# lisqzqng/Video-based-gait-analysis-for-dementia

Measured on AMD Instinct MI355X. Metric: frames/sec (224x224, seq=16), higher is better.
Workload: dtype f32

## Files before the change

video-based-gait-analysis-for-dementia_amd/csrc/conv_wino4.hip:

```cpp
#include "kernels.h"
#include "device.h"
#include "conv_wino4_tile.h"

#include <cstdio>
#include <cstdlib>

namespace grk {

namespace {

#ifdef GRNET_ABLATION
__device__ unsigned long long g_w4phase[8];
#endif

constexpr int kCK = 8;
constexpr size_t kLdsB = Wino4Geom<56, kCK, 256>::lds_bytes;

template <typename T>
__device__ __forceinline__ void landed(T& x) { asm volatile("" : "+v"(x)); }

template <int NB, int WD, int ABL, bool WSPLIT>
__device__ __forceinline__ void conv_wino4_body(const ConvArgs& a) {
    constexpr bool PAIR = NB == 2 && !WSPLIT;
    constexpr int NLD = PAIR ? 9 : 18;
// ... 175 lines not shown
                    if (has_add) y += rcur[i];
                    if (a.relu) { y[0] = fmaxf(y[0], 0.f); y[1] = fmaxf(y[1], 0.f); y[2] = fmaxf(y[2], 0.f); y[3] = fmaxf(y[3], 0.f); }
                    *reinterpret_cast<f32x4*>(a.out + obase + i * WD) = y;
                }
            }
        }
    }
    ticks.mark(3);
    ticks.count(4);
    ticks.flush(GRK_ABL_COUNTERS(g_w4phase), tid == 0);
}

template <int NB, int WD = 56, int ABL = 0, bool WSPLIT = false>
__global__ __launch_bounds__(256) void conv_wino4_f32(const ConvArgs a) { conv_wino4_body<NB, WD, ABL, WSPLIT>(a); }

constexpr int kCKW = 16;
constexpr size_t kLdsW = Wino4Geom<56, kCKW, 512>::lds_bytes;

template <int WD, int NPW>
__device__ __forceinline__ void conv_wino4w_body(const ConvArgs& a) {
    typedef Wino4Geom<WD, kCKW, 512> G;
    constexpr int TPR = G::TPR, TRG = G::TRG, kRawW = G::RAWW, UPC = G::UPC, kVW = G::V, kMrow = G::MROW;
    constexpr int COUTW = 2 * NPW * 16;
    static_assert(NPW == 4 || NPW == 2, "geometry");
    typedef float bfrag __attribute__((ext_vector_type(NPW)));
    extern __shared__ __align__(16) float smem[];
    float* raw = smem;
    float* V = raw + G::VOFF;
    const int tid = threadIdx.x, lane = tid & 63, wave = __builtin_amdgcn_readfirstlane(tid >> 6), l15 = lane & 15, lq = lane >> 4;
    const int pg = wave & 3, hf = wave >> 2;

    const int id = blockIdx.x;
    int img, r, by;
    G::decode(a, id, img, r, by);
    const int co0 = by * COUTW + hf * (NPW * 16);
    const int wpos = NPW == 4 ? co0 : (co0 & ~63) + ((co0 >> 5) & 1) * 2;
    set_wave_prio(a.prio);
    const int HW = a.H * a.W;
    const float* inb = a.in + ((size_t)img * a.in_ctot + a.in_coff) * HW;
    const int g0 = (4 * TRG * r - 1) * WD;

    const __amdgpu_buffer_rsrc_t u_rsrc = buffer_rsrc(a.w, 36 * a.CinPad * a.CoutPad * 4), r_rsrc = buffer_rsrc(inb, a.Cin * HW * 4);
    const int ub = ((pg * 9 * a.CinPad + lq) * a.CoutPad + wpos + l15 * 4) * 4;
    const int u_point = a.CinPad * a.CoutPad * 4, u_kstep = 4 * a.CoutPad * 4, u_chunk = kCKW * a.CoutPad * 4;
    auto load_u = [&](int chunk, int q, int e) -> bfrag {
        const int soff = chunk * u_chunk + (3 * (q >> 1) + (e >> 1)) * u_point + (2 * (q & 1) + (e & 1)) * u_kstep;
        if constexpr (NPW == 4) return __builtin_bit_cast(bfrag, __builtin_amdgcn_raw_buffer_load_b128(u_rsrc, ub, soff, 0));
        else return __builtin_bit_cast(bfrag, __builtin_amdgcn_raw_buffer_load_b64(u_rsrc, ub, soff, 0));
    };
    int roff[G::NRU];
#pragma unroll
    for (int i = 0; i < G::NRU; ++i) {
        const int u = i * G::NT + tid, ch = u / UPC, k = u - ch * UPC, gi = g0 + 4 * k;
        const bool unit = u < kCKW * UPC, inside = gi >= 0 && gi < HW;
        roff[i] = unit && inside ? (ch * HW + gi) * 4 : -1;
        if (unit && !inside) {
            *reinterpret_cast<f32x4*>(raw + u * 4) = f32x4{0.f, 0.f, 0.f, 0.f};
// ... 10 lines not shown
    const int vpos = (hf * 18) * (kCKW * 16) + chn * 16 + slot;
    auto transform = [&](const float* rp, float* vp) {
        Wino4Patch<G> t;
        t.read(rp);
        t.halo(real);
        t.rows(hf);
        t.cols(vp);
    };

    f32x4 acc[9][NPW];
#pragma unroll
    for (int p = 0; p < 9; ++p)
#pragma unroll
        for (int n = 0; n < NPW; ++n) acc[p][n] = f32x4{0.f, 0.f, 0.f, 0.f};

    const int nchunks = a.CinPad / kCKW;
    bfrag bq[6];
    float av[2][6];
    auto load_a = [&](int buf, int q, int set) {
#pragma unroll
        for (int e = 0; e < 6; ++e) {
            const int p = pg * 9 + 3 * (q >> 1) + (e >> 1), ks = 2 * (q & 1) + (e & 1);
            av[set][e] = V[buf * kVW + p * (kCKW * 16) + (ks * 4 + lq) * 16 + l15];
        }
    };
    auto multiply = [&](int buf, int ch, bool more) {
        load_a(buf, 0, 0);
#pragma unroll
        for (int q = 0; q < 6; ++q) {
#pragma unroll
            for (int e = 0; e < 6; ++e) landed(av[q & 1][e]);
// ... 1 lines not shown
            if (q < 5) load_a(buf, q + 1, (q + 1) & 1);
            __builtin_amdgcn_sched_barrier(0);
#pragma unroll
            for (int e = 0; e < 6; ++e) {
                const int pi = 3 * (q >> 1) + (e >> 1);
#pragma unroll
                for (int n = 0; n < NPW; ++n) acc[pi][n] = __builtin_amdgcn_mfma_f32_16x16x4f32(av[q & 1][e], bq[e][n], acc[pi][n], 0, 0, 0);
                __builtin_amdgcn_sched_barrier(0);
                if (q < 5) bq[e] = load_u(ch, q + 1, e);
                else if (more) bq[e] = load_u(ch + 1, 0, e);
                __builtin_amdgcn_sched_barrier(0);
            }
        }
    };

    const bool has_add = a.n_add == 1;
    const int eh = tid >> 8;
    typename G::Epi ep;
    G::epi(tid & 255, r, a.H, ep);
    f32x4 radd[4] = {f32x4{0.f, 0.f, 0.f, 0.f}, f32x4{0.f, 0.f, 0.f, 0.f}, f32x4{0.f, 0.f, 0.f, 0.f}, f32x4{0.f, 0.f, 0.f, 0.f}};
    auto fetch_res = [&](int nt) {
        const int co = by * COUTW + eh * (NPW * 16) + nt * 16 + ep.ec;
        if (has_add && ep.on && co < a.Cout) G::fetch_res(radd, a, ep, img, co, HW);
    };

    issue_raw(0);
    if (nchunks > 1) issue_raw(1);
#pragma unroll
    for (int e = 0; e < 6; ++e) bq[e] = load_u(0, 0, e);
    asm volatile("s_waitcnt vmcnt(6)" ::: "memory");
    __syncthreads();
// ... 30 lines not shown
        }
        __syncthreads();
        const f32x4 rcur[4] = {radd[0], radd[1], radd[2], radd[3]};
        if (nt + 1 < NPW) fetch_res(nt + 1);
        if (ep.on) {
            const int co = by * COUTW + eh * (NPW * 16) + nt * 16 + ep.ec;
            if (co < a.Cout) {
                float s4[4][6];
#pragma unroll
                for (int j = 0; j < 6; ++j) {
                    float m[6];
#pragma unroll
                    for (int i = 0; i < 6; ++i) m[i] = Mr[((i * 6 + j) * 16 + ep.ec) * kMrow + ep.et];
                    at_f43(m, s4[0][j], s4[1][j], s4[2][j], s4[3][j]);
                }
                const float b = a.bias[co];
                const size_t obase = ((size_t)img * a.out_ctot + a.out_coff + co) * HW + ep.eorow * WD + 4 * ep.etx;
#pragma unroll
                for (int i = 0; i < 4; ++i) {
                    float y0, y1, y2, y3;
                    at_f43<true>(s4[i], y0, y1, y2, y3, b);
                    f32x4 y = f32x4{y0, y1, y2, y3};
                    if (has_add) y += rcur[i];
                    if (a.relu) { y[0] = fmaxf(y[0], 0.f); y[1] = fmaxf(y[1], 0.f); y[2] = fmaxf(y[2], 0.f); y[3] = fmaxf(y[3], 0.f); }
                    *reinterpret_cast<f32x4*>(a.out + obase + i * WD) = y;
                }
            }
        }
    }
}

template <int WD, int NPW>
__global__ __launch_bounds__(512) void conv_wino4w_f32(const ConvArgs a) { conv_wino4w_body<WD, NPW>(a); }

}

int conv_wino4_wide(int cout, int w) {
    static const int wide_env = GRNET_AB(WINO_WIDE, 1);
    if (w == 56) return cout % 128 == 0 ? ((wide_env & 1) ? 4 : 0) : cout == 64 ? ((wide_env & 8) ? 2 : 0) : 0;
    if (w == 28) return cout % 128 == 0 ? ((wide_env & 4) ? 4 : 0) : cout == 64 ? ((wide_env & 2) ? 2 : 0) : 0;
    return 0;
}
int conv_wino4_blocks(int cout, int w) { return (cout % 64 == 0 && !(w == 28 && cout == 64 && !conv_wino4_wide(cout, w))) ? 4 : 2; }

bool conv_wino4_eligible(int cin, int cout, int ks, int stride, int h, int w, int n_add) {
    return ks == 3 && stride == 1 && ((h == 56 && w == 56) || (h == 28 && w == 28)) && n_add <= 1 && cin % kCK == 0 && cout % 32 == 0 && cin >= 32;
}

static size_t wino4_lds() {
    static const size_t pad = (size_t)GRNET_AB(WINO_LDS_PAD, 0);
    return kLdsB + pad;
}

hipError_t conv_wino4_form(const ConvArgs& a, Wino4Form* f) {
    *f = Wino4Form{};
    f->nb = conv_wino4_blocks(a.Cout, a.W);
    if (!conv_wino4_eligible(a.Cin, a.Cout, a.ks, a.stride, a.H, a.W, a.n_add) || a.CinPad % kCK != 0 || a.CoutPad % (f->nb * 16) != 0) return hipErrorInvalidValue;
    if (a.n_add == 1 && a.add_shift[0] != 0) return hipErrorInvalidValue;
    const int npw = conv_wino4_wide(a.Cout, a.W);
    const bool wide = npw && a.CinPad % kCKW == 0 && a.CoutPad % (npw * 32) == 0 && !(a.dbg & 32);
    const int trg = wino4_tile_rows(a.W);
    f->waves = wide ? 8 : 4;
    f->npw = wide ? npw : 0;
    f->gx = a.N * (((a.H >> 2) + trg - 1) / trg);
    f->gy = a.CoutPad / (wide ? npw * 32 : f->nb * 16);
    f->xcd = f->gx % 8 == 0 && f->gx >= 16 ? 1 : 0;
    const int total = f->gx * f->gy;
    f->full = total;
    if (wide || f->nb == 2) return hipSuccess;
    static const int split_env = GRNET_AB(WINO_SPLIT, 1);
    int kCUs = 0;
    if (hipError_t e = device_cu_count(&kCUs); e != hipSuccess) return e;
    const int full = total / kCUs * kCUs, rest = total - full;
    if (split_env && full > 0 && rest > 0 && 2 * rest <= kCUs && (!f->xcd || full % 8 == 0)) {
        f->split = 1;
        f->full = full;
        f->rest = rest;
    }
    return hipSuccess;
}

static void apply_form(ConvArgs& a, const Wino4Form& f, int* n_launches) {
    a.gx = f.gx;
    a.gy = f.gy;
// ... 18 lines not shown
        }
    }
#endif
    if (f.nb == 2) return launch_k(conv_wino4_f32<2, WD>, dim3(total), dim3(256), kLdsB, s, a);
    if (f.split) {
        hipError_t e = launch_k(conv_wino4_f32<4, WD>, dim3(f.full), dim3(256), kLdsB, s, a);
        if (e != hipSuccess) return e;
        a.blk0 = f.full;
        a.wsplit = 1;
        if (n_launches) *n_launches = 2;
        return launch_k(conv_wino4_f32<2, WD, 0, true>, dim3(2 * f.rest), dim3(256), kLdsB, s, a);
    }
    return launch_k(conv_wino4_f32<4, WD>, dim3(total), dim3(256), kLdsB, s, a);
}

hipError_t launch_conv_wino4(ConvArgs a, hipStream_t s, int* n_launches) {
    static PerDeviceOnce attr;
    int dev = 0;
    if (hipError_t e = current_device(&dev); e != hipSuccess) return e;
    if (hipError_t e = once_per_device(attr, dev, [](int*) {
            hipError_t e = hipSuccess;
            const size_t l4 = wino4_lds();
            auto set = [&](auto kern, size_t lds) { if (e == hipSuccess) e = hipFuncSetAttribute(reinterpret_cast<const void*>(kern), hipFuncAttributeMaxDynamicSharedMemorySize, (int)lds); };
            set(conv_wino4_f32<4, 56>, l4); set(conv_wino4_f32<2, 56>, l4); set(conv_wino4_f32<4, 28>, l4); set(conv_wino4_f32<2, 28>, l4);
            set(conv_wino4_f32<2, 56, 0, true>, l4); set(conv_wino4_f32<2, 28, 0, true>, l4);
            set(conv_wino4w_f32<56, 4>, kLdsW); set(conv_wino4w_f32<56, 2>, kLdsW); set(conv_wino4w_f32<28, 4>, kLdsW); set(conv_wino4w_f32<28, 2>, kLdsW);
            return e;
        }); e != hipSuccess) return e;
    Wino4Form f;
    if (hipError_t e = conv_wino4_form(a, &f); e != hipSuccess) return e;
    if (f.waves == 8) {
        apply_form(a, f, n_launches);
        const dim3 grid(a.gx * a.gy);
        if (a.W == 56) return f.npw == 4 ? launch_k(conv_wino4w_f32<56, 4>, grid, dim3(512), kLdsW, s, a) : launch_k(conv_wino4w_f32<56, 2>, grid, dim3(512), kLdsW, s, a);
        return f.npw == 4 ? launch_k(conv_wino4w_f32<28, 4>, grid, dim3(512), kLdsW, s, a) : launch_k(conv_wino4w_f32<28, 2>, grid, dim3(512), kLdsW, s, a);
    }
#ifdef GRNET_ABLATION
    if (GRNET_AB_SET(W4_PHASES)) {
        a.dbg |= 8;
        const hipError_t e = a.W == 56 ? launch_wino4_w<56>(a, s, f, n_launches) : launch_wino4_w<28>(a, s, f, n_launches);
        unsigned long long h[8] = {};
        abl::take_counters(HIP_SYMBOL(g_w4phase), h, s);
        const double n = h[4] ? (double)h[4] : 1.0;
        fprintf(stderr, "[wino4 phases] %d->%d @%d N%d add %d nb %d wgs %llu: per WG ticks  prologue %.0f  first transform %.0f  chunk loop %.0f (%d chunks)  epilogue %.0f\n",
                a.Cin, a.Cout, a.W, a.N, a.n_add, f.nb, h[4], h[0] / n, h[1] / n, h[2] / n, a.CinPad / kCK, h[3] / n);
        return e;
    }
// ... 34 lines not shown
```

video-based-gait-analysis-for-dementia_amd/csrc/grnet_hooks.cpp:

```cpp
#include "grnet_impl.h"

namespace {

struct HookBuffers {
    std::vector<void*> ptrs;
    HookBuffers() = default;
    HookBuffers(const HookBuffers&) = delete;
    HookBuffers& operator=(const HookBuffers&) = delete;
    ~HookBuffers() { for (void* p : ptrs) (void)hipFree(p); }
    template <class T = void>
    T* alloc(size_t bytes) {
        void* p = nullptr;
        if (hipMalloc(&p, bytes) != hipSuccess) return nullptr;
        ptrs.push_back(p);
        return static_cast<T*>(p);
    }
};

template <class F, class E>
float timed_launches(hipStream_t s, int reps, F&& launch, E* err) {
    hipEvent_t e0 = nullptr, e1 = nullptr;
    if (hipEventCreate(&e0) != hipSuccess || hipEventCreate(&e1) != hipSuccess) {
        if (e0) (void)hipEventDestroy(e0);
        return -1.f;
// ... 197 lines not shown
    if (hipMemcpy(wd, wp.data(), wp.size() * 4, hipMemcpyHostToDevice) != hipSuccess ||
        hipMemcpy(bd, bp.data(), bp.size() * 4, hipMemcpyHostToDevice) != hipSuccess)
        return h->fail(GRNET_EHIP, "hipMemcpy of the test weights failed");
    const int pad = ks / 2;
    ConvArgs a{};
    a.in = in_dev; a.in_ctot = cin; a.in_coff = 0; a.N = n; a.Cin = cin; a.H = hgt; a.W = wid;
    a.Cout = cout; a.Ho = (hgt + 2 * pad - ks) / stride + 1; a.Wo = (wid + 2 * pad - ks) / stride + 1;
    a.out = out_dev; a.out_ctot = cout; a.out_coff = 0;
    a.w = wd; a.bias = bd; a.CinPad = cin_pad; a.CoutPad = cout_pad; a.ks = ks; a.stride = stride; a.relu = relu;
    if (add_dev) { a.n_add = 1; a.add[0] = add_dev; a.add_ctot[0] = cout; a.add_coff[0] = 0; a.add_shift[0] = 0; }
    a.zeros = h->zeros;
    if (const char* d = GRNET_AB_STR(CONV_DBG)) a.dbg = atoi(d);
    hipStream_t s = static_cast<hipStream_t>(stream);
    float* ud = nullptr;
    if (tile_hint == 2003) { tile_hint = 2001; a.dbg |= 32; }
    if (tile_hint == 2001) {
        if (!conv_wino4_eligible(cin, cout, ks, stride, hgt, wid, add_dev ? 1 : 0) || cin_pad % 8 != 0 || cout_pad % (cout % 64 == 0 ? 64 : 32) != 0)
            return h->fail(GRNET_EINVAL, "shape not eligible for the F(4x4,3x3) kernel");
        std::vector<double> wf((size_t)cout * cin * 9);
        for (size_t i = 0; i < wf.size(); ++i) wf[i] = w_host[i];
        std::vector<float> uw((size_t)36 * cin_pad * cout_pad);
        pack_wino4_weights(wf.data(), cout, cin, cin_pad, cout_pad, uw.data(), wid);
        if (!(ud = mem.alloc<float>(uw.size() * 4)) || hipMemcpy(ud, uw.data(), uw.size() * 4, hipMemcpyHostToDevice) != hipSuccess)
            return h->fail(GRNET_ENOMEM, "Winograd test weights");
        a.w = ud;
    }
    if (tile_hint == 3002 && !conv_pw_eligible(cin, cout, ks, stride, hgt, wid, add_dev ? 1 : 0))
        return h->fail(GRNET_EINVAL, "shape not eligible for the 1x1 kernel");
    if (tile_hint == 3001) {
        if (!conv_stem_eligible(cin, cout, ks, stride, hgt, wid, add_dev ? 1 : 0))
            return h->fail(GRNET_EINVAL, "shape not eligible for the stem kernel");
        std::vector<double> wf((size_t)cout * cin * 9);
        for (size_t i = 0; i < wf.size(); ++i) wf[i] = w_host[i];
        std::vector<float> sw(7 * 4 * 64);
        pack_stem_weights(wf.data(), sw.data());
        if (!(ud = mem.alloc<float>(sw.size() * 4)) || hipMemcpy(ud, sw.data(), sw.size() * 4, hipMemcpyHostToDevice) != hipSuccess)
            return h->fail(GRNET_ENOMEM, "stem test weights");
        a.w = ud;
    }
    int w4s_on = 0, w4s_ks = 0;
    if (tile_hint >= 2020 && tile_hint <= 2024) {
        w4s_on = 1; w4s_ks = tile_hint - 2020;
        if (!conv_wino4s_eligible(cin, cout, ks, stride, hgt, wid, add_dev ? 1 : 0))
            return h->fail(GRNET_EINVAL, "shape not eligible for the small-map F(4x4,3x3) kernel");
        std::vector<double> wf((size_t)cout * cin * 9);
        for (size_t i = 0; i < wf.size(); ++i) wf[i] = w_host[i];
        std::vector<float> uw((size_t)36 * cin * cout);
        pack_wino4r_weights(wf.data(), cout, cin, uw.data());
        if (!(ud = mem.alloc<float>(uw.size() * 4)) || hipMemcpy(ud, uw.data(), uw.size() * 4, hipMemcpyHostToDevice) != hipSuccess)
            return h->fail(GRNET_ENOMEM, "Winograd test weights");
        a.w = ud;
    }
    auto launch_one = [&]() {
        return w4s_on ? launch_conv_wino4s(a, s, w4s_ks) : tile_hint == 2001 ? launch_conv_wino4(a, s) : tile_hint == 3001 ? launch_conv_stem(a, s) : tile_hint == 3002 ? launch_conv_pw(a, s) : launch_conv(a, s, tile_hint);
    };
    hipError_t e = launch_one();
    if (const char* r = GRNET_AB_STR(CONV_REPS)) {
        const int reps = atoi(r);
        const float ms = timed_launches(s, reps, launch_one, &e);
        fprintf(stderr, "[conv_micro] cin %d cout %d k %d s %d hw %d n %d hint %d dbg %d: %.2f us/launch\n", cin, cout, ks, stride, hgt, n,
                tile_hint, a.dbg, ms * 1e3f / reps);
    }
    hipError_t e2 = hipStreamSynchronize(s);
    if (e != hipSuccess) return h->fail(GRNET_EHIP, std::string("launch_conv: ") + hipGetErrorString(e));
    if (e2 != hipSuccess) return h->fail(GRNET_EHIP, std::string("conv kernel: ") + hipGetErrorString(e2));
    return 0;
}

int grnet_op_conv_chain(grnet_t* h, const float* in_dev, int n, int c, int wid, int nconv, const float* w_host, const float* bias_host, float* out_dev,
// ... 31 lines not shown
```

video-based-gait-analysis-for-dementia_amd/csrc/grnet_impl.h:

```cpp
#pragma once
#include "../../include/grnet_hip.h"

#include <hip/hip_runtime.h>

#include <cmath>
#include <cstdio>
#include <cstdlib>
#include <algorithm>
#include <cstring>
#include <map>
#include <memory>
#include <string>
#include <tuple>
#include <unordered_map>
#include <vector>

#include "kernels.h"

namespace grnet_detail {
using namespace grk;

inline uint16_t f32_to_bf16(float f) {
    uint32_t u;
    memcpy(&u, &f, 4);
// ... 14 lines not shown

struct ConvLayer {
    View in, out;
    std::vector<ConvSeg> segs;
    int cout = 0, ks = 1, stride = 1, relu = 0;
    int relu_from = 0;
    bool solo = false;
    int cin_w = 0;
    std::vector<AddRef> adds;
    float* w_dev = nullptr;
    float* b_dev = nullptr;
    float* wino4_dev = nullptr;
    float* stem_dev = nullptr;
    float* wino4s_dev = nullptr;
    int cin_pad = 0, cout_pad = 0;
    double macs_per_frame = 0;
    int lane_hint = 0;
    View in2;
    ConvSeg seg2;
    int pair_next = -1, pair_of = -1;
    int chain = -1, chain_pos = 0;
    int roll = -1, roll_pos = 0;
    std::map<int, int> tuned;
};

struct FuseUpPlan {
    int nb = 0;
    std::string prefix;
    std::vector<View> xs;
    std::vector<View> outs;
// ... 202 lines not shown
    View add_conv(View in, std::vector<ConvSeg> segs, int ks, int stride, bool relu, std::vector<AddRef> adds = {}, const View* out_override = nullptr);
    View conv_bn(View in, const std::string& wkey, const std::string& bn, int cout, int ks, int stride, bool relu, std::vector<AddRef> adds = {},
                 const View* out_override = nullptr);
    View add_bilinear(View in);
    std::vector<View> hr_module(std::vector<View> xs, const std::string& p, const View* out0);
    std::vector<View> hr_fuse_grouped(const std::vector<View>& xs, const std::string& p, const View* out0, const std::vector<int>& branch_tail);
    std::vector<View> hr_fuse_separate(std::vector<View> xs, const std::string& p, const View* out0, bool up0 = false, const std::vector<int>& branch_tail = {});
    void add_roll(int kind, int n_convs);
    void build_plan();
    void op_reads(const Op& op, std::vector<int>& r) const;
    void op_writes(const Op& op, std::vector<int>& w) const;
    void annotate_plan();
    std::string op_label(const Op& op) const;
    std::vector<std::vector<int>> launch_groups() const;
    int plan_arena(bool compact_layout, ArenaPlan& ap) const;
    void arena_info(const ArenaPlan& ap, int64_t* info) const;
    std::string arena_text(const ArenaPlan& ap) const;
    void schedule_lanes(std::vector<Op>& list, int n) const;
    void analyze_dependencies(std::vector<Op>& ops, std::vector<hipEvent_t>& op_events);

    const HostTensor* find(const std::string& k) const;
    int upload(const std::vector<float>& h, float** d);
    int upload_key(const std::string& k, size_t numel, const float** d);
    int pack_conv(ConvLayer& L);
    int pack_fuse_up(FuseUpPlan& fp);
    int finalize_gru();
    int finalize_tsattn();
    int finalize_featcorr();
    int finalize();

// ... 61 lines not shown
```

video-based-gait-analysis-for-dementia_amd/csrc/grnet_plan.cpp:

```cpp
#include "grnet_impl.h"
#include "lane_deps.h"

View grnet::new_buffer(int c, int h, int w) {
    const int ct = dtype == 1 ? (c + 7) / 8 * 8 : c;
    View v;
    v.slot = (int)buffer_floats.size();
    v.ctot = ct; v.coff = 0; v.c = c; v.h = h; v.w = w;
    buffer_floats.push_back((size_t)ct * h * w);
    return v;
}

View grnet::add_conv(View in, std::vector<ConvSeg> segs, int ks, int stride, bool relu, std::vector<AddRef> adds,
                     const View* out_override) {
    ConvLayer L;
    L.in = in;
    int cout = 0;
    for (auto& s : segs) cout += s.cout;
    const int pad = ks / 2;
    const int ho = (in.h + 2 * pad - ks) / stride + 1, wo = (in.w + 2 * pad - ks) / stride + 1;
    L.out = out_override ? *out_override : new_buffer(cout, ho, wo);
    L.segs = std::move(segs);
    L.cout = cout; L.ks = ks; L.stride = stride; L.relu = relu;
    L.adds = std::move(adds);
    L.cin_w = (dtype == 1 && in.c == 8 && in.ctot == 8) ? 3 : in.c;
// ... 395 lines not shown
    View part_feats = conv_bn(slice(first, 0, 128), hd + "keypoint_deconv_layers.3.weight", hd + "keypoint_deconv_layers.4", 128, 3, 1, true);
    name_view("head.part_feats", part_feats);
    v_heat = add_conv(part_feats, {ConvSeg{hd + "keypoint_final_layer.weight", "", hd + "keypoint_final_layer.bias", 25}}, 1, 1, false);
    name_view("head.heat", v_heat);
    cur_lane = 1;
    v_smpl_feats = conv_bn(slice(first, 128, 128), hd + "smpl_deconv_layers.3.weight", hd + "smpl_deconv_layers.4", 128, 3, 1, true);
    name_view("head.smpl_feats", v_smpl_feats);
    v_csmap = add_conv(v_smpl_feats, {ConvSeg{hd + "smpl_final_layer.weight", "", hd + "smpl_final_layer.bias", 64}}, 1, 1, false);
    name_view("head.cam_shape", v_csmap);
    cur_lane = 0;
    solo_region = false;
    Op op;
    op.kind = Op::POOL; ops.push_back(op);
    op.kind = Op::TAIL; ops.push_back(op);
    op.kind = Op::SMPL; ops.push_back(op);
    annotate_plan();
}

void grnet::op_reads(const Op& op, std::vector<int>& r) const {
    r.clear();
    auto put = [&](const View& v) { if (v.slot >= 0) r.push_back(v.slot); };
    switch (op.kind) {
        case Op::CONV: {
            const ConvLayer& L = convs[op.conv_idx];
            put(L.in);
            if (L.in2.c) put(L.in2);
            for (auto& a : L.adds) put(a.v);
            break;
        }
        case Op::SUM:
// ... 3 lines not shown
        case Op::FUSEUP:
        {
            const FuseUpPlan& fp = fuse_ups[op.conv_idx];
            for (size_t j = fp.only < 0 ? 0 : fp.only; j < fp.xs.size(); ++j) put(fp.xs[j]);
            for (size_t i = 0; i < fp.extra.size(); ++i)
                if (fp.only < 0 || fp.only == (int)i) for (auto& v : fp.extra[i]) put(v);
        }
            break;
        case Op::POOL: put(v_heat); put(v_smpl_feats); put(v_csmap); break;
        default: break;
    }
}
void grnet::op_writes(const Op& op, std::vector<int>& w) const {
    w.clear();
    auto put = [&](const View& v) { if (v.slot >= 0) w.push_back(v.slot); };
    if (op.kind == Op::CONV) put(convs[op.conv_idx].out);
    else if (op.kind == Op::SUM) put(sum_views[op.conv_idx].out);
    else if (op.kind == Op::BILINEAR) put(op.bout);
    else if (op.kind == Op::CONVERT) put(v_in8);
    else if (op.kind == Op::FUSEUP) {
        const FuseUpPlan& fp = fuse_ups[op.conv_idx];
        for (size_t i = 0; i < fp.outs.size(); ++i) if (fp.only < 0 || fp.only == (int)i) put(fp.outs[i]);
    }
}
void grnet::annotate_plan() {
    for (Op& op : ops) { op_reads(op, op.rd); op_writes(op, op.wr); }
    end_reads = {v_cat.slot, v_heat.slot, v_smpl_feats.slot};
}

std::string grnet::op_label(const Op& op) const {
    switch (op.kind) {
// ... 318 lines not shown
```

video-based-gait-analysis-for-dementia_amd/csrc/grnet_run.cpp:

```cpp
#include "grnet_impl.h"

namespace grk { thread_local GraphRecorder* g_recorder = nullptr; }

int grnet::allocate() {
    if (plan_arena(compact, arena_plan)) return fail(GRNET_ESTATE, "the activation arena could not be planned: a launch group or the assignment violates the sharing rule");
    const size_t total = (size_t)arena_plan.total;
    arena_floats = total;
    void* q = nullptr;
    if (hipMalloc(&q, total * sizeof(float)) != hipSuccess)
        return fail(GRNET_ENOMEM, std::string("hipMalloc of the ") + (compact ? "compact " : "") + "activation arena (" + std::to_string(total * 4 >> 20) + " MiB) failed");
    arena = static_cast<float*>(q);
    if (hipMemset(arena, 0, 64 * sizeof(float)) != hipSuccess) return fail(GRNET_EHIP, "hipMemset failed");
    zeros = arena;
    if (hipEventCreateWithFlags(&ev_fork, hipEventDisableTiming) != hipSuccess) return fail(GRNET_EHIP, "hipEventCreate failed");
    if (int rc = install_schedule(max_frames)) return rc;
    if (hipStreamCreateWithFlags(&capture_stream, hipStreamNonBlocking) != hipSuccess) return fail(GRNET_EHIP, "hipStreamCreate failed");
    const size_t n = max_frames;
    int rc;
    if ((rc = dev_alloc(&d_plf, n * 128 * 24))) return rc;
    if ((rc = dev_alloc(&d_csf, n * 64 * 24))) return rc;
    if ((rc = dev_alloc(&d_stats, softmax_pool_ws_floats((int)n)))) return rc;
    if ((rc = dev_alloc(&d_rot6d, n * 144))) return rc;
    if ((rc = dev_alloc(&d_shape, n * 10))) return rc;
    if ((rc = dev_alloc(&d_cam, n * 3))) return rc;
    if ((rc = dev_alloc(&d_rotmat, n * 216))) return rc;
    if ((rc = dev_alloc(&d_theta, n * 85))) return rc;
    if ((rc = dev_alloc(&d_A, n * kSmplWsFloatsPerFrame))) return rc;
    if ((rc = dev_alloc(&d_verts, n * 6890 * 3))) return rc;
    if ((rc = dev_alloc(&d_kp3d, n * 87))) return rc;
    if ((rc = dev_alloc(&d_kp2d, n * 58))) return rc;
    return 0;
}

int grnet::install_schedule(int n) {
    drop_graphs();
    seen_once.clear();
    for (hipEvent_t e : op_events_flat) if (e) (void)hipEventDestroy(e);
    op_events_flat.clear();
    ops_flat = ops;
    static const int sched_env = GRNET_AB(LANE_SCHED, 1);
    if (sched_env) schedule_lanes(ops_flat, n);
    analyze_dependencies(ops_flat, op_events_flat);
    int used = 1;
    for (const Op& op : ops_flat) used = std::max(used, op.lane + 1);
    for (int l = 1; l < used; ++l) {
// ... 88 lines not shown
int grnet::launch_form(const ConvLayer& L, int n, std::string* out) {
    char b[192];
    ConvArgs a = conv_args(L, nullptr, n);
    switch (kernel_for(L, n)) {
        case K_WINO4S: {
            const int ipw = conv_wino4s_images_per_tile(L.in.w);
            int last = 0;
            const int tiles = conv_wino4s_row_tiles(L.in.w, n, &last);
            snprintf(b, sizeof b, "wino4s images_per_tile=%d row_tiles=%d partial=%d", ipw, tiles, last < ipw ? 1 : 0);
            break;
        }
        case K_PW: snprintf(b, sizeof b, "pw"); break;
        case K_STEM: snprintf(b, sizeof b, "stem"); break;
        case K_WINO4: {
            Wino4Form f;
            if (conv_wino4_form(a, &f) != hipSuccess) return fail(GRNET_EINVAL, "no F(4x4,3x3) launch for " + L.segs[0].wkey);
            if (f.waves == 8) snprintf(b, sizeof b, "wino4w waves=8 npw=%d gx=%d gy=%d xcd=%d split=0", f.npw, f.gx, f.gy, f.xcd);
            else snprintf(b, sizeof b, "wino4 waves=4 nb=%d gx=%d gy=%d xcd=%d split=%d full=%d rest=%d", f.nb, f.gx, f.gy, f.xcd, f.split, f.full, f.rest);
            break;
        }
        case K_DIRECT: {
            const int hint = hint_for(L, n);
            ConvChoice c;
            if (conv_choose(a, hint, &c) != hipSuccess)
                return fail(GRNET_EINVAL, "tile hint " + std::to_string(hint) + " is not valid for " + L.segs[0].wkey + " at " + std::to_string(n) + " frames");
            snprintf(b, sizeof b, "direct split_k=%d pixel_tile=%d channel_tile=%d waves=%d width_variant=%d rows=%d hint=%d", c.family, c.tps * 16, c.tcs * 16,
                     c.waves, c.width_variant, c.rows, hint);
            break;
        }
        default: return fail(GRNET_ESTATE, "not an fp32 launch");
    }
    *out = b;
    return 0;
}
bool grnet::tap_written(const View& v) const {
    for (const ConvLayer& L : convs) {
        if (L.out.slot != v.slot || L.out.coff != v.coff || L.out.c != v.c) continue;
        switch (kernel_for(L, last_n)) {
            case K_BF16_ROLL: case K_BF16_ROLL_MEMBER: return L.roll_pos == (int)rolls[L.roll].convs.size() - 1;
            case K_BF16_CHAIN: case K_BF16_CHAIN_MEMBER: return L.chain_pos == (int)chains[L.chain].convs.size() - 1;
            default: return true;
        }
    }
    return true;
}

ConvArgs grnet::conv_args(const ConvLayer& L, const float* frames, int n) const {
    ConvArgs a{};
    bind(L.in, a.in, a.in_ctot, a.in_coff, frames);
    a.N = n; a.Cin = L.in.c; a.H = L.in.h; a.W = L.in.w;
    bind(L.out, a.out, a.out_ctot, a.out_coff);
    a.Cout = L.cout; a.Ho = L.out.h; a.Wo = L.out.w;
    a.w = L.w_dev; a.bias = L.b_dev; a.CinPad = L.cin_pad; a.CoutPad = L.cout_pad;
    a.ks = L.ks; a.stride = L.stride; a.relu = L.relu; a.relu_from = L.relu_from;
    a.n_add = (int)L.adds.size();
    for (int k = 0; k < a.n_add; ++k) {
        bind(L.adds[k].v, a.add[k], a.add_ctot[k], a.add_coff[k]);
        a.add_shift[k] = L.adds[k].shift;
    }
    a.zeros = zeros;
    a.pw_stream = !(chain_mode & 128) ? 0 : bf16_min_frames ? 2 : 1;
// ... 51 lines not shown
            HIP_TRY(launch_conv_wino4s(wa, s, w4s_ks));
            break;
        }
        case K_PW: HIP_TRY(launch_conv_pw(conv_args(L, frames, n), s)); break;
        case K_STEM: {
            ConvArgs wa = conv_args(L, frames, n);
            wa.w = L.stem_dev;
            HIP_TRY(launch_conv_stem(wa, s));
            break;
        }
        case K_WINO4: {
            ConvArgs wa = conv_args(L, frames, n);
            wa.w = L.wino4_dev;
            static const int chain_prio4 = GRNET_AB(WINO_PRIO, 1);
            wa.prio = (L.in.c == L.cout && L.cout <= 64 && !L.solo) ? chain_prio4 : 0;
            HIP_TRY(launch_conv_wino4(wa, s, n_launches));
            break;
        }
        case K_DIRECT: HIP_TRY(launch_conv(conv_args(L, frames, n), s, hint_for(L, n))); break;
    }
    return 0;
}
int grnet::launch_fuse_up_op(const FuseUpPlan& fp, int n, hipStream_t s) {
    FuseUpArgs a{};
    a.N = n; a.nb = fp.nb; a.only = fp.only;
    for (int i = 0; i < fp.nb - 1; ++i) {
        if (fp.only >= 0 && fp.only != i) continue;
        FuseUpOut& fo = a.o[i];
        bind(fp.outs[i], fo.out, fo.out_ctot, fo.out_coff);
        bind(fp.xs[i], fo.base, fo.base_ctot, fo.base_coff);
        fo.bias = fp.b_dev[i];
// ... 454 lines not shown
```

video-based-gait-analysis-for-dementia_amd/csrc/kernels.h:

```cpp
#pragma once
#include <hip/hip_runtime.h>
#include <stdint.h>
#include "raster_lines.h"

#include <initializer_list>
#include <mutex>
#include <string>
#include <tuple>
#include <utility>
#include <vector>

#ifdef GRNET_ABLATION
#include <cstdlib>
#define GRNET_AB(name, dflt) (getenv("GRNET_" #name) ? atoi(getenv("GRNET_" #name)) : (dflt))
#define GRNET_AB_F(name, dflt) (getenv("GRNET_" #name) ? atof(getenv("GRNET_" #name)) : (dflt))
#define GRNET_AB_SET(name) (getenv("GRNET_" #name) != nullptr)
#define GRNET_AB_STR(name) getenv("GRNET_" #name)
#else
#define GRNET_AB(name, dflt) (dflt)
#define GRNET_AB_F(name, dflt) (dflt)
#define GRNET_AB_SET(name) false
#define GRNET_AB_STR(name) (static_cast<const char*>(nullptr))
#endif

// ... 111 lines not shown
    int gx, gy, gx8, xcd;
    int pw_stream;
    int dbg;
    int prio;
    int blk0, wsplit;
};

hipError_t launch_conv(ConvArgs a, hipStream_t s, int tile_hint = 0);
struct ConvChoice { int family = 0, tps = 0, tcs = 0, nw = 0, waves = 0, width_variant = 0, rows = 0; };
hipError_t conv_choose(const ConvArgs& a, int tile_hint, ConvChoice* out);
int conv_pick_tc(int Cout);
hipError_t conv_init();
const char* conv_dominant_kernel_name();

bool conv_wino4_eligible(int cin, int cout, int ks, int stride, int h, int w, int n_add);
hipError_t launch_conv_wino4(ConvArgs a, hipStream_t s, int* n_launches = nullptr);
void pack_wino4_weights(const double* w_folded , int cout, int cin, int cin_pad, int cout_pad, float* out, int map_width = 56);
int conv_wino4_blocks(int cout, int map_width);
int conv_wino4_wide(int cout, int map_width);
struct Wino4Form { int waves = 0, nb = 0, npw = 0, gx = 0, gy = 0, xcd = 0, split = 0, full = 0, rest = 0; };
hipError_t conv_wino4_form(const ConvArgs& a, Wino4Form* f);

void wino4_transform_filter(const double* g33, double* u36);
bool conv_pw_eligible(int cin, int cout, int ks, int stride, int h, int w, int n_add);
hipError_t launch_conv_pw(ConvArgs a, hipStream_t s);
bool conv_stem_eligible(int cin, int cout, int ks, int stride, int h, int w, int n_add);
hipError_t launch_conv_stem(ConvArgs a, hipStream_t s);
void pack_stem_weights(const double* w_folded , float* out );
bool conv_wino4s_eligible(int cin, int cout, int ks, int stride, int h, int w, int n_add);
hipError_t launch_conv_wino4s(ConvArgs a, hipStream_t s, int ksplit);
int conv_wino4s_images_per_tile(int map_width);
int conv_wino4s_row_tiles(int map_width, int n_images, int* last_tile_images);
void pack_wino4r_weights(const double* w_folded , int cout, int cin, float* out );
struct SumArgs {
    float* out; int out_ctot, out_coff;
    int N, C, H, W, relu, n_add;
// ... 302 lines not shown
```

Before: 4564.

## Split the Winograd tail wave along input channels with atomic-counter reduction

For 56x56 wide Winograd convolutions whose workgroup count leaves a partial last round on the CUs, the leftover units are split into two pieces along the input-channel chunks, chosen by a cost model. Each piece writes partial output tiles to a workspace. The second piece to finish, detected through an atomic counter, sums both partials, adds bias and relu, and writes the output. This targets the tail-wave load imbalance, at the cost of extra workspace traffic, an atomic per unit and a larger grid.

New measurement: 4580, median of 6. Within noise of the previous version (+0.3%).

```diff
diff --git a/video-based-gait-analysis-for-dementia_amd/csrc/conv_wino4.hip b/video-based-gait-analysis-for-dementia_amd/csrc/conv_wino4.hip
--- a/video-based-gait-analysis-for-dementia_amd/csrc/conv_wino4.hip
+++ b/video-based-gait-analysis-for-dementia_amd/csrc/conv_wino4.hip
@@ -1,6 +1,7 @@
 #include "kernels.h"
 #include "device.h"
 #include "conv_wino4_tile.h"
+#include "conv_wino4_ksplit.h"
 
 #include <cstdio>
 #include <cstdlib>
@@ -213,33 +214,65 @@
 template <int NB, int WD = 56, int ABL = 0, bool WSPLIT = false>
 __global__ __launch_bounds__(256) void conv_wino4_f32(const ConvArgs a) { conv_wino4_body<NB, WD, ABL, WSPLIT>(a); }
 
+static_assert(kWino4KCounters == kWino4KMaxCut, "a layer's counters cover the largest cut");
 constexpr int kCKW = 16;
 constexpr size_t kLdsW = Wino4Geom<56, kCKW, 512>::lds_bytes;
 
-template <int WD, int NPW>
-__device__ __forceinline__ void conv_wino4w_body(const ConvArgs& a) {
+struct Wino4KArgs { float* ws; unsigned* cnt; int whole, cut, k0, rev, rw; };
+
+template <int WD, int NPW, bool KS = false>
+__device__ __forceinline__ void conv_wino4w_body(const ConvArgs& a, const Wino4KArgs& kk) {
+    static_assert(!KS || (WD == 56 && NPW == 4), "the cut is built for the 128-channel workgroups of the 56-wide maps");
     typedef Wino4Geom<WD, kCKW, 512> G;
     constexpr int TPR = G::TPR, TRG = G::TRG, kRawW = G::RAWW, UPC = G::UPC, kVW = G::V, kMrow = G::MROW;
     constexpr int COUTW = 2 * NPW * 16;
+    [[maybe_unused]] constexpr size_t kSlotW = wino4_ksplit_slot_floats();
     static_assert(NPW == 4 || NPW == 2, "geometry");
     typedef float bfrag __attribute__((ext_vector_type(NPW)));
+    typedef unsigned u32x4k __attribute__((ext_vector_type(4)));
     extern __shared__ __align__(16) float smem[];
     float* raw = smem;
     float* V = raw + G::VOFF;
     const int tid = threadIdx.x, lane = tid & 63, wave = __builtin_amdgcn_readfirstlane(tid >> 6), l15 = lane & 15, lq = lane >> 4;
     const int pg = wave & 3, hf = wave >> 2;
 
-    const int id = blockIdx.x;
+    int id = blockIdx.x;
+    [[maybe_unused]] int kb = 0, ke = 0, part = -1;
+    if constexpr (KS) {
+        const int blk = kk.rev ? (int)gridDim.x - 1 - (int)blockIdx.x : (int)blockIdx.x;
+        const Wino4KPiece pc = wino4_ksplit_piece(kk.whole, kk.cut, kk.k0, a.CinPad / kCKW, blk);
+        id = __builtin_amdgcn_readfirstlane(pc.unit);
+        kb = __builtin_amdgcn_readfirstlane(pc.k_begin);
+        ke = __builtin_amdgcn_readfirstlane(pc.k_end);
+        part = __builtin_amdgcn_readfirstlane(pc.part);
+    }
     int img, r, by;
-    G::decode(a, id, img, r, by);
+    if constexpr (KS) {
+        const int rows = part < 0 ? kk.rw : 14 - kk.rw, r0 = part < 0 ? 0 : kk.rw, u = part < 0 ? id : id - kk.whole, gxp = a.N * rows;
+        int bx;
+        if (gxp % 8 == 0 && gxp >= 16) {
+            const int j = u >> 3, x = u & 7, q = j / a.gy;
+            by = j - q * a.gy;
+            bx = x * (gxp >> 3) + q;
+        } else {
+            bx = u / a.gy;
+            by = u - bx * a.gy;
+        }
+        img = bx / rows;
+        r = r0 + bx - img * rows;
+    } else {
+        G::decode(a, id, img, r, by);
+    }
     const int co0 = by * COUTW + hf * (NPW * 16);
     const int wpos = NPW == 4 ? co0 : (co0 & ~63) + ((co0 >> 5) & 1) * 2;
     set_wave_prio(a.prio);
     const int HW = a.H * a.W;
-    const float* inb = a.in + ((size_t)img * a.in_ctot + a.in_coff) * HW;
+    const float* inb = a.in + ((size_t)img * a.in_ctot + a.in_coff + (KS ? kb * kCKW : 0)) * HW;
     const int g0 = (4 * TRG * r - 1) * WD;
 
-    const __amdgpu_buffer_rsrc_t u_rsrc = buffer_rsrc(a.w, 36 * a.CinPad * a.CoutPad * 4), r_rsrc = buffer_rsrc(inb, a.Cin * HW * 4);
+    const __amdgpu_buffer_rsrc_t u_rsrc = KS ? buffer_rsrc(a.w + (size_t)kb * kCKW * a.CoutPad, (36 * a.CinPad - kb * kCKW) * a.CoutPad * 4)
+                                             : buffer_rsrc(a.w, 36 * a.CinPad * a.CoutPad * 4),
+                                 r_rsrc = buffer_rsrc(inb, (a.Cin - (KS ? kb * kCKW : 0)) * HW * 4);
     const int ub = ((pg * 9 * a.CinPad + lq) * a.CoutPad + wpos + l15 * 4) * 4;
     const int u_point = a.CinPad * a.CoutPad * 4, u_kstep = 4 * a.CoutPad * 4, u_chunk = kCKW * a.CoutPad * 4;
     auto load_u = [&](int chunk, int q, int e) -> bfrag {
@@ -280,7 +313,7 @@
 #pragma unroll
         for (int n = 0; n < NPW; ++n) acc[p][n] = f32x4{0.f, 0.f, 0.f, 0.f};
 
-    const int nchunks = a.CinPad / kCKW;
+    const int nchunks = KS ? ke - kb : a.CinPad / kCKW;
     bfrag bq[6];
     float av[2][6];
     auto load_a = [&](int buf, int q, int set) {
@@ -312,7 +345,7 @@
         }
     };
 
-    const bool has_add = a.n_add == 1;
+    const bool has_add = !KS && a.n_add == 1;
     const int eh = tid >> 8;
     typename G::Epi ep;
     G::epi(tid & 255, r, a.H, ep);
@@ -373,24 +406,73 @@
                     for (int i = 0; i < 6; ++i) m[i] = Mr[((i * 6 + j) * 16 + ep.ec) * kMrow + ep.et];
                     at_f43(m, s4[0][j], s4[1][j], s4[2][j], s4[3][j]);
                 }
-                const float b = a.bias[co];
-                const size_t obase = ((size_t)img * a.out_ctot + a.out_coff + co) * HW + ep.eorow * WD + 4 * ep.etx;
-#pragma unroll
-                for (int i = 0; i < 4; ++i) {
-                    float y0, y1, y2, y3;
-                    at_f43<true>(s4[i], y0, y1, y2, y3, b);
-                    f32x4 y = f32x4{y0, y1, y2, y3};
-                    if (has_add) y += rcur[i];
-                    if (a.relu) { y[0] = fmaxf(y[0], 0.f); y[1] = fmaxf(y[1], 0.f); y[2] = fmaxf(y[2], 0.f); y[3] = fmaxf(y[3], 0.f); }
-                    *reinterpret_cast<f32x4*>(a.out + obase + i * WD) = y;
+                if (KS && part >= 0) {
+                    const __amdgpu_buffer_rsrc_t w_rsrc = buffer_rsrc(kk.ws + ((size_t)(id - kk.whole) * 2 + part) * kSlotW, (int)(kSlotW * 4));
+                    const int wo = (((eh * (NPW * 16) + nt * 16 + ep.ec) * 4) * WD + 4 * ep.etx) * 4;
+#pragma unroll
+                    for (int i = 0; i < 4; ++i) {
+                        float y0, y1, y2, y3;
+                        at_f43<false>(s4[i], y0, y1, y2, y3);
+                        __builtin_amdgcn_raw_buffer_store_b128(__builtin_bit_cast(u32x4k, f32x4{y0, y1, y2, y3}), w_rsrc, wo + i * (WD * 4), 0, 16);
+                    }
+                } else {
+                    const float b = a.bias[co];
+                    const size_t obase = ((size_t)img * a.out_ctot + a.out_coff + co) * HW + ep.eorow * WD + 4 * ep.etx;
+#pragma unroll
+                    for (int i = 0; i < 4; ++i) {
+                        float y0, y1, y2, y3;
+                        at_f43<true>(s4[i], y0, y1, y2, y3, b);
+                        f32x4 y = f32x4{y0, y1, y2, y3};
+                        if (has_add) y += rcur[i];
+                        if (a.relu) { y[0] = fmaxf(y[0], 0.f); y[1] = fmaxf(y[1], 0.f); y[2] = fmaxf(y[2], 0.f); y[3] = fmaxf(y[3], 0.f); }
+                        *reinterpret_cast<f32x4*>(a.out + obase + i * WD) = y;
+                    }
                 }
             }
         }
     }
+    if constexpr (KS) {
+        if (part < 0) return;
+        unsigned* const arrived = reinterpret_cast<unsigned*>(smem + 2 * G::MTILE);
+        asm volatile("s_waitcnt vmcnt(0)" ::: "memory");
+        __syncthreads();
+        if (tid == 0) {
+            const unsigned before = __hip_atomic_fetch_add(kk.cnt + (id - kk.whole), 1u, __ATOMIC_RELAXED, __HIP_MEMORY_SCOPE_AGENT);
+            if (before == 1u) {
+                __builtin_amdgcn_fence(__ATOMIC_ACQUIRE, "agent");
+                asm volatile("s_waitcnt vmcnt(0)" ::: "memory");
+            }
+            *reinterpret_cast<volatile unsigned*>(arrived) = before;
+        }
+        __syncthreads();
+        if (*reinterpret_cast<volatile unsigned*>(arrived) != 1u) return;
+        const float* const p0 = kk.ws + (size_t)(id - kk.whole) * 2 * kSlotW;
+        if (ep.on) {
+#pragma unroll
+            for (int nt = 0; nt < NPW; ++nt) {
+                const int co = by * COUTW + eh * (NPW * 16) + nt * 16 + ep.ec;
+                if (co < a.Cout) {
+                    const float b = a.bias[co];
+                    const float* sp = p0 + ((eh * (NPW * 16) + nt * 16 + ep.ec) * 4) * WD + 4 * ep.etx;
+                    const size_t obase = ((size_t)img * a.out_ctot + a.out_coff + co) * HW + ep.eorow * WD + 4 * ep.etx;
+#pragma unroll
+                    for (int i = 0; i < 4; ++i) {
+                        const f32x4 first = *reinterpret_cast<const f32x4*>(sp + i * WD), second = *reinterpret_cast<const f32x4*>(sp + kSlotW + i * WD);
+                        f32x4 y = first + second;
+                        y += f32x4{b, b, b, b};
+                        if (a.relu) { y[0] = fmaxf(y[0], 0.f); y[1] = fmaxf(y[1], 0.f); y[2] = fmaxf(y[2], 0.f); y[3] = fmaxf(y[3], 0.f); }
+                        *reinterpret_cast<f32x4*>(a.out + obase + i * WD) = y;
+                    }
+                }
+            }
+        }
+        if (tid == 0) __hip_atomic_store(kk.cnt + (id - kk.whole), 0u, __ATOMIC_RELAXED, __HIP_MEMORY_SCOPE_AGENT);
+    }
 }
 
 template <int WD, int NPW>
-__global__ __launch_bounds__(512) void conv_wino4w_f32(const ConvArgs a) { conv_wino4w_body<WD, NPW>(a); }
+__global__ __launch_bounds__(512) void conv_wino4w_f32(const ConvArgs a) { conv_wino4w_body<WD, NPW>(a, Wino4KArgs{}); }
+__global__ __launch_bounds__(512) void conv_wino4wk_f32(const ConvArgs a, const Wino4KArgs kk) { conv_wino4w_body<56, 4, true>(a, kk); }
 
 }
 
@@ -411,7 +493,7 @@
     return kLdsB + pad;
 }
 
-hipError_t conv_wino4_form(const ConvArgs& a, Wino4Form* f) {
+hipError_t conv_wino4_form(const ConvArgs& a, Wino4Form* f, const Wino4KSplitWs* ks) {
     *f = Wino4Form{};
     f->nb = conv_wino4_blocks(a.Cout, a.W);
     if (!conv_wino4_eligible(a.Cin, a.Cout, a.ks, a.stride, a.H, a.W, a.n_add) || a.CinPad % kCK != 0 || a.CoutPad % (f->nb * 16) != 0) return hipErrorInvalidValue;
@@ -426,7 +508,31 @@
     f->xcd = f->gx % 8 == 0 && f->gx >= 16 ? 1 : 0;
     const int total = f->gx * f->gy;
     f->full = total;
-    if (wide || f->nb == 2) return hipSuccess;
+    if (wide) {
+        static const int ksplit_env = GRNET_AB(WINO_KSPLIT, 1);
+        if (!ks || !ks->ws || !ks->cnt || npw != 4 || a.W != 56 || a.H != 56 || a.n_add != 0 || !ksplit_env) return hipSuccess;
+        const int chunks = a.CinPad / kCKW;
+        Wino4KPlan p;
+        if (ks->force_k0 > 0) {
+            if (ks->force_k0 >= chunks) return hipErrorInvalidValue;
+            p.whole = 0; p.cut = total; p.k0 = ks->force_k0;
+        } else {
+            int cus = 0;
+            if (hipError_t e = device_cu_count(&cus); e != hipSuccess) return e;
+            static const double over_env = GRNET_AB_F(WINO_KSPLIT_OVER, -1.0);
+            static const int k0_env = GRNET_AB(WINO_KSPLIT_K0, 0);
+            const int group = a.N * f->gy;
+            p = over_env < 0 ? wino4_ksplit_plan(total, chunks, cus, a.n_add, group) : wino4_ksplit_plan(total, chunks, cus, a.n_add, group, kWino4KOverWhole, over_env, 0.0);
+            if (p.cut > 0 && k0_env > 0 && k0_env < chunks) p.k0 = k0_env;
+        }
+        if (p.cut > 0 && (size_t)p.cut * 2 * wino4_ksplit_slot_floats() <= ks->ws_floats && p.cut <= ks->cnt_words) {
+            f->kwhole = p.whole; f->kcut = p.cut; f->k0 = p.k0;
+            f->krows = p.whole / (a.N * f->gy);
+            f->krev = ks->force_k0 > 0 && ks->reverse ? 1 : 0;
+        }
+        return hipSuccess;
+    }
+    if (f->nb == 2) return hipSuccess;
     static const int split_env = GRNET_AB(WINO_SPLIT, 1);
     int kCUs = 0;
     if (hipError_t e = device_cu_count(&kCUs); e != hipSuccess) return e;
@@ -475,7 +581,7 @@
     return launch_k(conv_wino4_f32<4, WD>, dim3(total), dim3(256), kLdsB, s, a);
 }
 
-hipError_t launch_conv_wino4(ConvArgs a, hipStream_t s, int* n_launches) {
+hipError_t launch_conv_wino4(ConvArgs a, hipStream_t s, int* n_launches, const Wino4KSplitWs* ks) {
     static PerDeviceOnce attr;
     int dev = 0;
     if (hipError_t e = current_device(&dev); e != hipSuccess) return e;
@@ -486,12 +592,15 @@
             set(conv_wino4_f32<4, 56>, l4); set(conv_wino4_f32<2, 56>, l4); set(conv_wino4_f32<4, 28>, l4); set(conv_wino4_f32<2, 28>, l4);
             set(conv_wino4_f32<2, 56, 0, true>, l4); set(conv_wino4_f32<2, 28, 0, true>, l4);
             set(conv_wino4w_f32<56, 4>, kLdsW); set(conv_wino4w_f32<56, 2>, kLdsW); set(conv_wino4w_f32<28, 4>, kLdsW); set(conv_wino4w_f32<28, 2>, kLdsW);
+            set(conv_wino4wk_f32, kLdsW);
             return e;
         }); e != hipSuccess) return e;
     Wino4Form f;
-    if (hipError_t e = conv_wino4_form(a, &f); e != hipSuccess) return e;
+    if (hipError_t e = conv_wino4_form(a, &f, ks); e != hipSuccess) return e;
     if (f.waves == 8) {
         apply_form(a, f, n_launches);
+        if (f.kcut > 0)
+            return launch_k(conv_wino4wk_f32, dim3(f.kwhole + 2 * f.kcut), dim3(512), kLdsW, s, a, Wino4KArgs{ks->ws, ks->cnt, f.kwhole, f.kcut, f.k0, f.krev, f.krows});
         const dim3 grid(a.gx * a.gy);
         if (a.W == 56) return f.npw == 4 ? launch_k(conv_wino4w_f32<56, 4>, grid, dim3(512), kLdsW, s, a) : launch_k(conv_wino4w_f32<56, 2>, grid, dim3(512), kLdsW, s, a);
         return f.npw == 4 ? launch_k(conv_wino4w_f32<28, 4>, grid, dim3(512), kLdsW, s, a) : launch_k(conv_wino4w_f32<28, 2>, grid, dim3(512), kLdsW, s, a);
diff --git a/video-based-gait-analysis-for-dementia_amd/csrc/conv_wino4_ksplit.h b/video-based-gait-analysis-for-dementia_amd/csrc/conv_wino4_ksplit.h
--- /dev/null
+++ b/video-based-gait-analysis-for-dementia_amd/csrc/conv_wino4_ksplit.h
@@ -0,0 +1,56 @@
+#pragma once
+
+#if defined(__HIPCC__)
+#define WINO4K_HD __host__ __device__
+#else
+#define WINO4K_HD
+#endif
+
+namespace grk {
+
+constexpr int kWino4KMaxCut = 1024;
+constexpr double kWino4KOverWhole = 2.4, kWino4KOverPiece = 3.0, kWino4KOverFinish = 3.7, kWino4KMargin = 1.0;
+
+struct Wino4KPlan {
+    int whole = 0, cut = 0, k0 = 0;
+    double span_uncut = 0, span = 0;
+};
+
+inline double wino4_ksplit_tail(int rest, int cus, int chunks, int k0, double over_piece, double over_finish) {
+    const int others = cus - rest, turns = (rest + others - 1) / others;
+    const double first = k0 + over_piece + over_finish, second = turns * (chunks - k0 + over_piece);
+    return first > second ? first : second;
+}
+
+inline Wino4KPlan wino4_ksplit_plan(int units, int chunks, int cus, int n_add, int group = 1, double over_whole = kWino4KOverWhole,
+                                    double over_piece = kWino4KOverPiece, double over_finish = kWino4KOverFinish, double margin = kWino4KMargin) {
+    Wino4KPlan p;
+    p.whole = units;
+    if (units < 1 || chunks < 1 || cus < 1 || group < 1) return p;
+    const int rounds = (units + cus - 1) / cus, rest = units % cus;
+    p.span_uncut = p.span = rounds * (chunks + over_whole);
+    if (rest == 0 || n_add != 0 || chunks < 2 || rest > kWino4KMaxCut || rest % group != 0 || units % group != 0) return p;
+    int best_k0 = 0;
+    double best = 0;
+    for (int k0 = 1; k0 < chunks; ++k0) {
+        const double t = wino4_ksplit_tail(rest, cus, chunks, k0, over_piece, over_finish);
+        if (!best_k0 || t < best) { best = t; best_k0 = k0; }
+    }
+    const double span = (rounds - 1) * (chunks + over_whole) + best;
+    if (span + margin > p.span_uncut) return p;
+    p.whole = units - rest;
+    p.cut = rest;
+    p.k0 = best_k0;
+    p.span = span;
+    return p;
+}
+
+struct Wino4KPiece { int unit, k_begin, k_end, part; };
+WINO4K_HD inline Wino4KPiece wino4_ksplit_piece(int whole, int cut, int k0, int chunks, int block) {
+    if (block < whole) return Wino4KPiece{block, 0, chunks, -1};
+    const int t = block - whole;
+    if (t < cut) return Wino4KPiece{whole + t, 0, k0, 0};
+    return Wino4KPiece{whole + t - cut, k0, chunks, 1};
+}
+
+}
diff --git a/video-based-gait-analysis-for-dementia_amd/csrc/grnet_hooks.cpp b/video-based-gait-analysis-for-dementia_amd/csrc/grnet_hooks.cpp
--- a/video-based-gait-analysis-for-dementia_amd/csrc/grnet_hooks.cpp
+++ b/video-based-gait-analysis-for-dementia_amd/csrc/grnet_hooks.cpp
@@ -235,6 +235,13 @@
     hipStream_t s = static_cast<hipStream_t>(stream);
     float* ud = nullptr;
     if (tile_hint == 2003) { tile_hint = 2001; a.dbg |= 32; }
+    Wino4KSplitWs ksw;
+    bool never_cut = false;
+    if (tile_hint >= 2100 && tile_hint < 2300 && tile_hint != 2200) {
+        ksw.force_k0 = tile_hint % 100; ksw.reverse = tile_hint >= 2200;
+        never_cut = tile_hint == 2100;
+        tile_hint = 2001;
+    }
     if (tile_hint == 2001) {
         if (!conv_wino4_eligible(cin, cout, ks, stride, hgt, wid, add_dev ? 1 : 0) || cin_pad % 8 != 0 || cout_pad % (cout % 64 == 0 ? 64 : 32) != 0)
             return h->fail(GRNET_EINVAL, "shape not eligible for the F(4x4,3x3) kernel");
@@ -245,6 +252,14 @@
         if (!(ud = mem.alloc<float>(uw.size() * 4)) || hipMemcpy(ud, uw.data(), uw.size() * 4, hipMemcpyHostToDevice) != hipSuccess)
             return h->fail(GRNET_ENOMEM, "Winograd test weights");
         a.w = ud;
+        if (conv_wino4_wide(cout, wid) == 4 && wid == 56 && !add_dev && !never_cut) {
+            const int units = n * 14 * (cout_pad / 128);
+            ksw.ws_floats = (size_t)units * 2 * wino4_ksplit_slot_floats();
+            ksw.cnt_words = units;
+            ksw.ws = mem.alloc<float>(ksw.ws_floats * 4);
+            ksw.cnt = mem.alloc<unsigned>((size_t)units * 4);
+            if (!ksw.ws || !ksw.cnt || hipMemset(ksw.cnt, 0, (size_t)units * 4) != hipSuccess) return h->fail(GRNET_ENOMEM, "Winograd cut workspace");
+        }
     }
     if (tile_hint == 3002 && !conv_pw_eligible(cin, cout, ks, stride, hgt, wid, add_dev ? 1 : 0))
         return h->fail(GRNET_EINVAL, "shape not eligible for the 1x1 kernel");
@@ -273,7 +288,7 @@
         a.w = ud;
     }
     auto launch_one = [&]() {
-        return w4s_on ? launch_conv_wino4s(a, s, w4s_ks) : tile_hint == 2001 ? launch_conv_wino4(a, s) : tile_hint == 3001 ? launch_conv_stem(a, s) : tile_hint == 3002 ? launch_conv_pw(a, s) : launch_conv(a, s, tile_hint);
+        return w4s_on ? launch_conv_wino4s(a, s, w4s_ks) : tile_hint == 2001 ? launch_conv_wino4(a, s, nullptr, &ksw) : tile_hint == 3001 ? launch_conv_stem(a, s) : tile_hint == 3002 ? launch_conv_pw(a, s) : launch_conv(a, s, tile_hint);
     };
     hipError_t e = launch_one();
     if (const char* r = GRNET_AB_STR(CONV_REPS)) {
diff --git a/video-based-gait-analysis-for-dementia_amd/csrc/grnet_impl.h b/video-based-gait-analysis-for-dementia_amd/csrc/grnet_impl.h
--- a/video-based-gait-analysis-for-dementia_amd/csrc/grnet_impl.h
+++ b/video-based-gait-analysis-for-dementia_amd/csrc/grnet_impl.h
@@ -52,6 +52,8 @@
     float* stem_dev = nullptr;
     float* wino4s_dev = nullptr;
     int cin_pad = 0, cout_pad = 0;
+    View ksplit_ws;
+    unsigned* ksplit_cnt = nullptr;
     double macs_per_frame = 0;
     int lane_hint = 0;
     View in2;
@@ -284,6 +286,7 @@
     std::string op_label(const Op& op) const;
     std::vector<std::vector<int>> launch_groups() const;
     int plan_arena(bool compact_layout, ArenaPlan& ap) const;
+    Wino4KSplitWs ksplit_of(const ConvLayer& L) const;
     void arena_info(const ArenaPlan& ap, int64_t* info) const;
     std::string arena_text(const ArenaPlan& ap) const;
     void schedule_lanes(std::vector<Op>& list, int n) const;
diff --git a/video-based-gait-analysis-for-dementia_amd/csrc/grnet_plan.cpp b/video-based-gait-analysis-for-dementia_amd/csrc/grnet_plan.cpp
--- a/video-based-gait-analysis-for-dementia_amd/csrc/grnet_plan.cpp
+++ b/video-based-gait-analysis-for-dementia_amd/csrc/grnet_plan.cpp
@@ -433,6 +433,10 @@
     op.kind = Op::POOL; ops.push_back(op);
     op.kind = Op::TAIL; ops.push_back(op);
     op.kind = Op::SMPL; ops.push_back(op);
+    if (dtype == 0)
+        for (ConvLayer& L : convs)
+            if (L.ks == 3 && L.stride == 1 && L.in.h == 56 && L.in.w == 56 && L.adds.empty() && L.cout >= 256 && L.cout % 128 == 0 && L.in.c % 16 == 0)
+                L.ksplit_ws = new_buffer(2 * L.cout, 56, 56);
     annotate_plan();
 }
 
@@ -466,7 +470,7 @@
 void grnet::op_writes(const Op& op, std::vector<int>& w) const {
     w.clear();
     auto put = [&](const View& v) { if (v.slot >= 0) w.push_back(v.slot); };
-    if (op.kind == Op::CONV) put(convs[op.conv_idx].out);
+    if (op.kind == Op::CONV) { put(convs[op.conv_idx].out); put(convs[op.conv_idx].ksplit_ws); }
     else if (op.kind == Op::SUM) put(sum_views[op.conv_idx].out);
     else if (op.kind == Op::BILINEAR) put(op.bout);
     else if (op.kind == Op::CONVERT) put(v_in8);
diff --git a/video-based-gait-analysis-for-dementia_amd/csrc/grnet_run.cpp b/video-based-gait-analysis-for-dementia_amd/csrc/grnet_run.cpp
--- a/video-based-gait-analysis-for-dementia_amd/csrc/grnet_run.cpp
+++ b/video-based-gait-analysis-for-dementia_amd/csrc/grnet_run.cpp
@@ -29,6 +29,13 @@
     if ((rc = dev_alloc(&d_verts, n * 6890 * 3))) return rc;
     if ((rc = dev_alloc(&d_kp3d, n * 87))) return rc;
     if ((rc = dev_alloc(&d_kp2d, n * 58))) return rc;
+    for (ConvLayer& L : convs) {
+        if (L.ksplit_ws.slot < 0) continue;
+        float* q = nullptr;
+        if ((rc = dev_alloc(&q, kWino4KCounters))) return rc;
+        if (hipMemset(q, 0, kWino4KCounters * sizeof(unsigned)) != hipSuccess) return fail(GRNET_EHIP, "hipMemset failed");
+        L.ksplit_cnt = reinterpret_cast<unsigned*>(q);
+    }
     return 0;
 }
 
@@ -147,8 +154,9 @@
         case K_STEM: snprintf(b, sizeof b, "stem"); break;
         case K_WINO4: {
             Wino4Form f;
-            if (conv_wino4_form(a, &f) != hipSuccess) return fail(GRNET_EINVAL, "no F(4x4,3x3) launch for " + L.segs[0].wkey);
-            if (f.waves == 8) snprintf(b, sizeof b, "wino4w waves=8 npw=%d gx=%d gy=%d xcd=%d split=0", f.npw, f.gx, f.gy, f.xcd);
+            const Wino4KSplitWs ks = ksplit_of(L);
+            if (conv_wino4_form(a, &f, &ks) != hipSuccess) return fail(GRNET_EINVAL, "no F(4x4,3x3) launch for " + L.segs[0].wkey);
+            if (f.waves == 8) snprintf(b, sizeof b, "wino4w waves=8 npw=%d gx=%d gy=%d xcd=%d split=0 kwhole=%d kcut=%d k0=%d", f.npw, f.gx, f.gy, f.xcd, f.kwhole, f.kcut, f.k0);
             else snprintf(b, sizeof b, "wino4 waves=4 nb=%d gx=%d gy=%d xcd=%d split=%d full=%d rest=%d", f.nb, f.gx, f.gy, f.xcd, f.split, f.full, f.rest);
             break;
         }
@@ -178,6 +186,15 @@
     return true;
 }
 
+Wino4KSplitWs grnet::ksplit_of(const ConvLayer& L) const {
+    Wino4KSplitWs ks;
+    if (L.ksplit_ws.slot < 0 || !L.ksplit_cnt) return ks;
+    ks.ws = base(L.ksplit_ws);
+    ks.ws_floats = buffer_floats[L.ksplit_ws.slot] * (size_t)max_frames;
+    ks.cnt = L.ksplit_cnt;
+    ks.cnt_words = kWino4KCounters;
+    return ks;
+}
 ConvArgs grnet::conv_args(const ConvLayer& L, const float* frames, int n) const {
     ConvArgs a{};
     bind(L.in, a.in, a.in_ctot, a.in_coff, frames);
@@ -259,7 +276,8 @@
             wa.w = L.wino4_dev;
             static const int chain_prio4 = GRNET_AB(WINO_PRIO, 1);
             wa.prio = (L.in.c == L.cout && L.cout <= 64 && !L.solo) ? chain_prio4 : 0;
-            HIP_TRY(launch_conv_wino4(wa, s, n_launches));
+            const Wino4KSplitWs ks = ksplit_of(L);
+            HIP_TRY(launch_conv_wino4(wa, s, n_launches, &ks));
             break;
         }
         case K_DIRECT: HIP_TRY(launch_conv(conv_args(L, frames, n), s, hint_for(L, n))); break;
diff --git a/video-based-gait-analysis-for-dementia_amd/csrc/kernels.h b/video-based-gait-analysis-for-dementia_amd/csrc/kernels.h
--- a/video-based-gait-analysis-for-dementia_amd/csrc/kernels.h
+++ b/video-based-gait-analysis-for-dementia_amd/csrc/kernels.h
@@ -149,12 +149,16 @@
 const char* conv_dominant_kernel_name();
 
 bool conv_wino4_eligible(int cin, int cout, int ks, int stride, int h, int w, int n_add);
-hipError_t launch_conv_wino4(ConvArgs a, hipStream_t s, int* n_launches = nullptr);
+struct Wino4KSplitWs;
+hipError_t launch_conv_wino4(ConvArgs a, hipStream_t s, int* n_launches = nullptr, const Wino4KSplitWs* ks = nullptr);
 void pack_wino4_weights(const double* w_folded , int cout, int cin, int cin_pad, int cout_pad, float* out, int map_width = 56);
 int conv_wino4_blocks(int cout, int map_width);
 int conv_wino4_wide(int cout, int map_width);
-struct Wino4Form { int waves = 0, nb = 0, npw = 0, gx = 0, gy = 0, xcd = 0, split = 0, full = 0, rest = 0; };
-hipError_t conv_wino4_form(const ConvArgs& a, Wino4Form* f);
+struct Wino4Form { int waves = 0, nb = 0, npw = 0, gx = 0, gy = 0, xcd = 0, split = 0, full = 0, rest = 0, kwhole = 0, kcut = 0, k0 = 0, krev = 0, krows = 0; };
+struct Wino4KSplitWs { float* ws = nullptr; size_t ws_floats = 0; unsigned* cnt = nullptr; int cnt_words = 0; int force_k0 = 0, reverse = 0; };
+constexpr int kWino4KCounters = 1024;
+constexpr size_t wino4_ksplit_slot_floats() { return 128 * 4 * 56; }
+hipError_t conv_wino4_form(const ConvArgs& a, Wino4Form* f, const Wino4KSplitWs* ks = nullptr);
 
 void wino4_transform_filter(const double* g33, double* u36);
 bool conv_pw_eligible(int cin, int cout, int ks, int stride, int h, int w, int n_add);
```
